# kisasexypantera94/hpfw

Hardware: AMD Instinct MI355X
Metric: hashprints/sec (index) + Hamming matches/sec (search), 30 s@44.1 kHz clips (higher is better)
Workload: dtype f32 (transforms, dB) + int8 digits / int64 sums (projection); 1 GPU; configs[1]: 1000 x 30 s synthetic 44.1 kHz PCM16 clips per GPU, hashprint extraction only (CQT + dB + projection + bit pack), inputs resident in HBM; clips_per_gpu=1000, hashprints_per_clip=2320, parallelism=clips sharded over 1 GPU(s), no collective on this path

## Files before the change

hpfw_amd/csrc/extract.hip:

```cpp
#include "handle.h"

int pass_clips(hpfw_gpu *h, const DevPlan *dp, int64_t n_clips)
{
    const hpfw::HostPlan &p = dp->hp;
    size_t per_clip = (size_t)121 * p.c * 4 + (size_t)64 * std::max(p.n_frames, 1) * 4;
    if (p.bluestein)
        per_clip += 2 * hpfw::bz_plane_bytes(dp->bz, 1) + (size_t)(p.kmax - p.kmin) * 8;
    else
        per_clip += (size_t)hpfw::z_floats_per_clip(p.hq, p.n2) * 4 + (size_t)p.n1 * p.q2w * 8;
    size_t work = 0;
    for (const hpfw::CqClassDev &cd : dp->cls) work = std::max(work, hpfw::cq_big_work_bytes(cd, 1));
    per_clip += work;
    const int64_t fit = std::max<int64_t>(1, (int64_t)(((size_t)24 << 30) / per_clip));
    const int64_t cap = std::min<int64_t>(h->batch, fit), n = std::max<int64_t>(n_clips, 1);
    const int64_t passes = (n + cap - 1) / cap;
    return (int)((n + passes - 1) / passes);
}

int ensure_ws(hpfw_gpu *h, const DevPlan *dp, int nb, int ns)
{
    const hpfw::HostPlan &p = dp->hp;
    size_t work = 0;
    for (const hpfw::CqClassDev &cd : dp->cls) work = std::max(work, hpfw::cq_big_work_bytes(cd, nb));
    if (work) {
// ... 196 lines not shown
{
    *use = nullptr;
    if (n_shifts || h->q_products != 6 || !h->projection) return 0;
    const int64_t tiles = hpfw::project_q_tiles(n_clips, c);
    if (tiles <= 0) return 0;
    if (int rc = ensure(h->d_q_split, hpfw::project_q_split_bytes(tiles, h->q_fixup_launch), h)) return rc;
    *qs = {h->d_q_thr.as<int32_t>(), h->d_q_split.get(), h->q_fixup_launch ? h->d_fq32.as<int32_t>() : nullptr};
    *use = qs;
    return 0;
}

namespace {
int run_back(hpfw_gpu *h, DevPlan *dp, const void *images, int n_shifts, int ns, uint64_t *d_hp, hipStream_t s)
{
    const hpfw::HostPlan &p = dp->hp;
    const float *sdb = h->ws[2].as<float>();
    int rc;
    if (h->projection) {
        hpfw::QSplit qs;
        const hpfw::QSplit *split;
        if ((rc = q_split(h, n_shifts, ns, p.c, &qs, &split))) return rc;
        {
            Timed t(h, K_PROJECT, s);
            hpfw::launch_hashprints_q(images, n_shifts, sdb, h->d_clipmax.as<float>(), ns, p.c, d_hp, nullptr, s, split);
        }
        if (split) h->q_last_tiles = hpfw::project_q_tiles(ns, p.c);
        return check_launch("project");
    }
    float *proj = h->ws[3].as<float>();
    {
        Timed t(h, K_PROJECT, s);
        hpfw::launch_project(h->d_fpack.as<float>(), sdb, h->d_clipmax.as<float>(), ns, p.c, proj, s);
    }
    if ((rc = check_launch("project"))) return rc;
    {
        Timed t(h, K_PACK, s);
        hpfw::launch_pack(proj, ns, p.n_frames, d_hp, s);
    }
    return check_launch("delta_pack");
}

constexpr int kBackBatch = 1024;

int check_filters(const hpfw_gpu *h) { return h->has_filters ? 0 : fail(HPFW_E_NOFILTERS, "no filters: call hpfw_gpu_set_filters or hpfw_gpu_learn_filters first"); }

int check_shifts(const int32_t *shifts, int n_shifts)
{
// ... 30 lines not shown
    if ((rc = check_filters(h))) return rc;
    return 0;
}

int hashprints_from_db(hpfw_gpu *h, const float *d_db, int64_t n_clips, int64_t c, const int32_t *shifts, int n_shifts, uint64_t *d_hp,
                       hipStream_t s)
{
    const int64_t nf = c - (hpfw::kCtx - 1), nhp = nf - hpfw::kLag;
    HIP_TRY(hipSetDevice(h->device));
    return ordered_call(h, s, [&] {
        int rc;
        if (n_shifts && (rc = shift_images(h, shifts, n_shifts, s))) return rc;
        const void *images = n_shifts ? h->d_shift_images.get() : h->d_fq_image.get();
        const int nbmax = 256;
        if (!h->projection && (rc = ensure(h->ws[3], (size_t)nbmax * 64 * (size_t)nf * 4))) return rc;
        hpfw::QSplit qs;
        const hpfw::QSplit *split;
        if ((rc = q_split(h, n_shifts, std::min<int64_t>(nbmax, n_clips), c, &qs, &split))) return rc;
        for (int64_t c0 = 0; c0 < n_clips; c0 += nbmax) {
            const int nb = (int)std::min<int64_t>(nbmax, n_clips - c0);
            if (h->projection) {
                Timed t(h, K_PROJECT, s);
                hpfw::launch_hashprints_q(images, n_shifts, d_db + c0 * 121 * c, nullptr, nb, (int)c, d_hp + c0 * std::max(n_shifts, 1) * nhp,
                                          nullptr, s, split);
                if (split) h->q_last_tiles = hpfw::project_q_tiles(nb, c);
            } else {
                hpfw::launch_project(h->d_fpack.as<float>(), d_db + c0 * 121 * c, nullptr, nb, (int)c, h->ws[3].as<float>(), s);
                hpfw::launch_pack(h->ws[3].as<float>(), nb, (int)nf, d_hp + c0 * nhp, s);
            }
            if ((rc = check_launch("project"))) return rc;
        }
        return 0;
    });
}

constexpr size_t kTempoBudget = (size_t)256 << 20;

int check_tempos(const float *tempos, int n_tempos, int n_shifts)
{
    if (!tempos || n_tempos < 1 || n_tempos > hpfw::kMaxTempos) return fail(HPFW_E_INVALID, "tempos: 1 to 64 values");
    for (int i = 0; i < n_tempos; ++i) {
        if (!(tempos[i] >= 0.5f && tempos[i] <= 2.0f)) return fail(HPFW_E_INVALID, "tempos: finite values in [0.5, 2]");
        for (int j = 0; j < i; ++j)
            if (hpfw::tempo_step(tempos[j]) == hpfw::tempo_step(tempos[i]))
                return fail(HPFW_E_INVALID, "tempos: values must have distinct steps rint(65536 / tempo)");
    }
    if ((int64_t)n_tempos * std::max(n_shifts, 1) > hpfw::kMaxShifts) return fail(HPFW_E_INVALID, "tempos x shifts: at most 64 variants");
// ... 20 lines not shown
    return ct;
}

int tempo_back(hpfw_gpu *h, const void *images, int n_shifts, const float *d_db, int64_t nb, int64_t c, const hpfw::TempoList &tl,
               int64_t ct, uint64_t *d_hp, hipStream_t s)
{
    const int64_t per_pair = (int64_t)std::max(n_shifts, 1) * (ct - (hpfw::kCtx - 1) - hpfw::kLag);
    const size_t pair_bytes = (size_t)hpfw::kBins * ct * 4;
    const int64_t pairs = std::max<int64_t>(1, (int64_t)(kTempoBudget / pair_bytes));
    const int64_t cb = pairs >= tl.n ? std::min<int64_t>(pairs / tl.n, nb) : 1;
    const int tb = pairs >= tl.n ? tl.n : (int)pairs;
    int rc;
    if ((rc = ensure(h->d_tempo, (size_t)cb * tb * pair_bytes, h))) return rc;
    float *scaled = h->d_tempo.as<float>();
    for (int64_t c0 = 0; c0 < nb; c0 += cb) {
        const int nc = (int)std::min(cb, nb - c0);
        for (int j0 = 0; j0 < tl.n; j0 += tb) {
            hpfw::TempoList sub{std::min(tb, tl.n - j0), {}};
            for (int j = 0; j < sub.n; ++j) sub.step[j] = tl.step[j0 + j];
            hpfw::launch_tempo_scale(d_db + c0 * hpfw::kBins * c, nc, c, sub, ct, scaled, s);
            if ((rc = check_launch("tempo_scale"))) return rc;
            {
                Timed t(h, K_PROJECT, s);
                hpfw::launch_hashprints_q(images, n_shifts, scaled, nullptr, nc * sub.n, (int)ct, d_hp + (c0 * tl.n + j0) * per_pair, nullptr, s);
            }
            if ((rc = check_launch("project"))) return rc;
        }
    }
    return 0;
}

int extract_tempo_pcm16(hpfw_gpu *h, const int16_t *d_pcm, int64_t n_samples, int64_t n_clips, const float *tempos, int n_tempos,
                        const int32_t *shifts, int n_shifts, uint64_t *d_hp, void *stream)
{
    hpfw::TempoList tl;
    int rc = check_tempo_call(h, tempos, n_tempos, shifts, n_shifts, &tl);
    if (rc) return rc;
    if (!d_pcm || !d_hp || n_clips < 0) return fail(HPFW_E_INVALID, "bad argument");
    HIP_TRY(hipSetDevice(h->device));
    DevPlan *dp;
    if ((rc = get_plan(h, n_samples, &dp))) return rc;
    const int64_t c = dp->hp.c, ct = tempo_common_columns(c, tl);
    if (ct - (hpfw::kCtx - 1) - hpfw::kLag < 1) return fail(HPFW_E_UNSUPPORTED, "clip too short to yield a hashprint at the slowest tempo");
    if (n_clips == 0) return 0;
    const int64_t per_clip = (int64_t)tl.n * std::max(n_shifts, 1) * (ct - (hpfw::kCtx - 1) - hpfw::kLag);
    hipStream_t s = (hipStream_t)stream;
    return ordered_call(h, s, [&] {
// ... 105 lines not shown
    *tiles = h->q_last_tiles;
    for (uint32_t v : counts) {
        if (v == 0xffffffffu) *redone += 1;
        else *listed += v;
    }
    return 0;
}

int hpfw_gpu_stage_delta_q(hpfw_gpu *h, const float *d_db, int64_t n_clips, int64_t c, int64_t *d_delta, uint64_t *d_hp, void *stream)
{
    if (!h || !d_db || !d_delta) return fail(HPFW_E_INVALID, "null argument");
    if (int rc = check_filters(h)) return rc;
    const int64_t nhp = c - (hpfw::kCtx - 1) - hpfw::kLag;
    if (nhp <= 0 || n_clips <= 0) return 0;
    if (n_clips > 65535) return fail(HPFW_E_INVALID, "at most 65535 clips per call");
    HIP_TRY(hipSetDevice(h->device));
    hipStream_t s = (hipStream_t)stream;
    return ordered_call(h, s, [&] {
        uint64_t *hp = d_hp;
        if (!hp) {
            if (int rc = ensure(h->ws[3], (size_t)n_clips * (size_t)nhp * 8)) return rc;
            hp = h->ws[3].as<uint64_t>();
        }
        hpfw::launch_hashprints_q(h->d_fq_image.get(), 0, d_db, nullptr, (int)n_clips, (int)c, hp, (long long *)d_delta, s);
        return check_launch("project");
    });
}

int hpfw_gpu_hashprints_from_db_transposed(hpfw_gpu *h, const float *d_db, int64_t n_clips, int64_t c, const int32_t *shifts,
                                           int n_shifts, uint64_t *d_hp, void *stream)
{
    int rc = check_transposed(h, shifts, n_shifts);
    if (rc) return rc;
    if (!d_db || !d_hp || n_clips < 0) return fail(HPFW_E_INVALID, "bad argument");
    if (c - (hpfw::kCtx - 1) - hpfw::kLag <= 0 || n_clips == 0) return 0;
    return hashprints_from_db(h, d_db, n_clips, c, shifts, n_shifts, d_hp, (hipStream_t)stream);
}

int hpfw_gpu_extract_pcm16(hpfw_gpu *h, const int16_t *d_pcm, int64_t n_samples, int64_t n_clips,
                           uint64_t *d_hp, void *stream)
{
    return extract_pcm16(h, d_pcm, n_samples, n_clips, nullptr, 0, d_hp, stream);
}

int hpfw_gpu_extract_transposed_pcm16(hpfw_gpu *h, const int16_t *d_pcm, int64_t n_samples, int64_t n_clips, const int32_t *shifts,
                                      int n_shifts, uint64_t *d_hp, void *stream)
{
// ... 440 lines not shown
```

hpfw_amd/csrc/handle.h:

```cpp
#pragma once
#include <hip/hip_runtime.h>

#include <algorithm>
#include <cstdio>
#include <cstdlib>
#include <cstring>
#include <condition_variable>
#include <chrono>
#include <map>
#include <memory>
#include <mutex>
#include <set>
#include <string>
#include <vector>

#include "../../include/hpfw_gpu.h"
#include "combiner.h"
#include "hip_owned.h"
#include "kernels.h"
#include "legacy_internal.h"
#include "plan.h"

using hpfw::DevBuf, hpfw::Event, hpfw::HostBuf, hpfw::Stream;

// ... 29 lines not shown
struct PlanTiming;

enum KernelKind { K_ROWS = 0, K_COLS, K_CQ, K_DB, K_PROJECT, K_PACK, K_SCAN, K_TOPK, K_PAIRS, K_FWD, K_COUNT };

struct TimedLaunch {
    int kind;
    Event a, b;
};

struct CallStatus {
    int rc = 0;
    std::string msg;
};

struct hpfw_gpu {
    int device = 0;
    bool has_filters = false;
    std::vector<float> filters;
    DevBuf d_fpack;
    DevBuf d_fq_image;
    DevBuf d_q_thr, d_fq32, d_q_split;
    int q_products = 6;
    bool q_fixup_launch = false;
    int64_t q_last_tiles = 0;
    int projection = 1;
    struct PlanCache {
        PlanCache();
        ~PlanCache();
        std::multimap<size_t, DevBuf> dev_pool;
        size_t dev_pool_bytes = 0;
        std::map<int64_t, std::unique_ptr<DevPlan>> plans;
        std::mutex host_mtx;
        std::condition_variable host_cv;
        std::map<int64_t, std::unique_ptr<hpfw::HostPlan>> host_ready;
        std::set<int64_t> host_seen;
        size_t plan_bytes = 0;
        uint64_t plan_clock = 0;
        uint64_t idle_clock = 0;
        std::unique_ptr<PlanTiming> plan_timing;
        Stream plan_stream;
        HostBuf pin_ring;
        size_t pin_off = 0;
        Event plan_ev;
        bool plan_ev_pending = false;
    } cache;
    unsigned conventions = 0;
// ... 179 lines not shown
```

hpfw_amd/csrc/handle.hip:

```cpp
#include "handle.h"

namespace {
thread_local std::string g_err;

const char *const kKernelNames[K_COUNT] = {"fwd_rows", "fwd_cols", "cq_chirpz", "db",
                                           "project_mfma", "delta_pack", "hamming_scan", "topk", "pcm_pairs", "fwd_span"};
}

int fail(int code, const std::string &msg)
{
    g_err = msg;
    return code;
}

extern "C" {

const char *hpfw_gpu_last_error(void) { return g_err.c_str(); }
void hpfw_internal_set_error(const char *msg) { g_err = msg ? msg : ""; }
const char *hpfw_gpu_version(void) { return "hpfw-gpu 0.1 (gfx950)"; }

int hpfw_gpu_create(int device, hpfw_gpu **out)
{
    if (!out) return fail(HPFW_E_INVALID, "out is NULL");
    *out = nullptr;
    int n = 0;
    HIP_TRY(hipGetDeviceCount(&n));
    if (device < 0 || device >= n) return fail(HPFW_E_INVALID, "no such device");
    HIP_TRY(hipSetDevice(device));
    auto h = std::make_unique<hpfw_gpu>();
    h->device = device;
    if (std::getenv("HPFW_CQ_SERIAL")) h->cq_concurrent = 0;
    if (const char *e = std::getenv("HPFW_FWD_CHUNK")) h->fwd_chunk = std::max(0, atoi(e));
    if (const char *e = std::getenv("HPFW_BZ_CHUNK")) h->bz_chunk = std::max(0, atoi(e));
    if (const char *e = std::getenv("HPFW_COLS_VARIANT")) h->cols_variant = atoi(e);
    if (const char *e = std::getenv("HPFW_PRUNE")) h->prune = (unsigned)std::strtoul(e, nullptr, 0);
    if (const char *e = std::getenv("HPFW_Q_PRODUCTS")) h->q_products = atoi(e) == 9 ? 9 : 6;
    if (const char *e = std::getenv("HPFW_Q_FIXUP")) h->q_fixup_launch = std::strcmp(e, "launch") == 0;
    if (const char *e = std::getenv("HPFW_DB_TERM")) h->db_fast = std::strcmp(e, "spec") != 0;
    if (const char *e = std::getenv("HPFW_FWD_STREAMS")) h->fwd_streams = std::min(hpfw_gpu::kCqSide + 1, std::max(1, atoi(e)));
    if (const char *e = std::getenv("HPFW_PROJECTION"))
        h->projection = std::strcmp(e, "f32") == 0 ? 0 : 1;
    if (h->ev0.create(hipEventDefault) != hipSuccess || h->ev1.create(hipEventDefault) != hipSuccess || h->order_ev.create() != hipSuccess ||
        init_plans(h.get()) != hipSuccess)
        return fail(HPFW_E_HIP, "hipEventCreate failed");
    *out = h.release();
    return 0;
}

int hpfw_gpu_device(const hpfw_gpu *h) { return h ? h->device : -1; }

void hpfw_gpu_destroy(hpfw_gpu *h)
{
    if (!h) return;
    (void)hipSetDevice(h->device);
    (void)hipDeviceSynchronize();
    delete h;
}

int hpfw_gpu_set_filters(hpfw_gpu *h, const float *f)
{
// ... 111 lines not shown
```

hpfw_amd/csrc/k_project_q.hip:

```cpp
#include <algorithm>
#include <cmath>
#include <cstdint>
#include <cstdlib>
#include <vector>

#include "kernels.h"

namespace hpfw {

extern __shared__ __align__(16) unsigned char smem_raw[];

typedef int v4i __attribute__((ext_vector_type(4)));
typedef int v16i __attribute__((ext_vector_type(16)));

constexpr int kQThreads = 256;
constexpr int kQTileN = 128;
constexpr int kQCols = kQTileN + kCtx - 1;
constexpr int kQPitch = 160;
constexpr int kQChunks = 8;
constexpr int kQUnit = 48;
constexpr int kQSlabBytes = kQChunks * kQPitch * kQUnit;
constexpr int kQStepBytes = 3 * 64 * 16;
constexpr int kQSteps = 2 * kCtx;
constexpr int kQLdsBytes = kQSlabBytes + kQTileN * 4 * 2;
constexpr float kQScale = 98304.0f;
constexpr int kQCap = 128;
constexpr unsigned kQRedo = 0xffffffffu;
constexpr int kQLdsBytes6 = kQLdsBytes + 16;
constexpr int kQLdsBytes6f = kQLdsBytes6 + kQCap * 2;

__device__ __forceinline__ unsigned q_digit_bytes(int u) { return ((unsigned)u + 0x808080u) ^ 0x808080u; }

__device__ __forceinline__ int q_fixed(float s)
{
    return (int)__builtin_rintf(__builtin_fminf(__builtin_fmaxf(s, -80.0f), 0.0f) * kQScale);
}

__device__ __forceinline__ long long q_value_from_digits(const v4i *__restrict__ fq_image, const unsigned char *slab, int r, int nl, int lane)
{
    constexpr int kPairs = 4 * kQSteps;
    v4i fa[3][3], sb[3][3];
#pragma unroll
    for (int k = 0; k < 3; ++k) {
        const int pair = min(lane + 64 * k, kPairs - 1);
        const int s = pair >> 2, g = pair & 3;
        const v4i *fu = fq_image + ((size_t)(r >> 4) * kQSteps + s) * (kQStepBytes / 16) + (r & 15) + 16 * g;
        const v4i *su = reinterpret_cast<const v4i *>(slab + (size_t)((4 * (s & 1) + g) * kQPitch + nl + (s >> 1)) * kQUnit);
#pragma unroll
        for (int d = 0; d < 3; ++d) {
            fa[k][d] = fu[d * 64];
            sb[k][d] = su[d];
        }
    }
    if (lane + 128 >= kPairs) sb[2][0] = sb[2][1] = sb[2][2] = v4i{0, 0, 0, 0};
    int acc[5] = {0, 0, 0, 0, 0};
#pragma unroll
    for (int k = 0; k < 3; ++k)
#pragma unroll
        for (int i = 0; i < 3; ++i)
#pragma unroll
            for (int j = 0; j < 3; ++j)
#pragma unroll
                for (int w = 0; w < 4; ++w) acc[i + j] = __builtin_amdgcn_sdot4(fa[k][i][w], sb[k][j][w], acc[i + j], false);
    long long v = acc[4];
#pragma unroll
    for (int cls = 3; cls >= 0; --cls) v = v * 256 + acc[cls];
#pragma unroll
    for (int m = 32; m >= 1; m >>= 1) v += __shfl_xor(v, m);
    return v;
}

template <bool FROM_T, bool SHIFTED, int NP, bool FUSED = false, bool STAGED = false>
__device__ __forceinline__ void hashprint_q_tile(const unsigned t, const v4i *__restrict__ fq_images, const float *__restrict__ sdb,
                                                 const float *__restrict__ tmax, int c, int nhp, int n_tiles_x, uint64_t *__restrict__ hp,
                                                 long long *__restrict__ dbg, int n_images, const int *__restrict__ thr,
                                                 unsigned *__restrict__ counts, unsigned short *__restrict__ seg)
{
    static_assert(NP == 9 || (NP == 6 && !SHIFTED), "six products: the extraction's unshifted image only");
    static_assert((!FUSED || NP == 6) && (!STAGED || (NP == 9 && !SHIFTED)), "FUSED: six products; STAGED: its nine-product redo");
    unsigned char *slab = smem_raw;
    unsigned short *parts = reinterpret_cast<unsigned short *>(smem_raw + kQSlabBytes);
    unsigned *n_open = reinterpret_cast<unsigned *>(smem_raw + kQLdsBytes);
    unsigned short *list = reinterpret_cast<unsigned short *>(smem_raw + kQLdsBytes6);
    const int tid = threadIdx.x, lane = tid & 63, wave = tid >> 6;
    const int kg = lane >> 4, cl = lane & 15;
    const int clip = t / n_tiles_x;
    const int n0 = (t - clip * n_tiles_x) * kQTileN;
    if (NP == 6 && tid == 0) *n_open = 0;
#if defined(HPFW_Q_STAMPS)
    long long st[6];
    st[0] = __builtin_amdgcn_s_memtime();
#define Q_STAMP(k) st[k] = __builtin_amdgcn_s_memtime()
#else
#define Q_STAMP(k) ((void)0)
#endif
    const float *S = sdb + (int64_t)clip * kBins * c;
    const float ref = FROM_T ? tmax[clip] : 0.0f;
    const v4i *img = fq_images + (size_t)wave * kQSteps * (kQStepBytes / 16) + lane;
    v4i a[3][3];
#pragma unroll
    for (int d = 0; d < 3; ++d) {
        a[0][d] = img[d * 64];
        a[1][d] = img[(kQStepBytes / 16) + d * 64];
    }
    constexpr int kUnits = (kQChunks * kQCols + kQThreads - 1) / kQThreads;
    unsigned any_digit = 0;
#pragma unroll 1
    for (int r0 = STAGED ? kUnits : 0; r0 < kUnits; r0 += 2) {
        float va[2][16], vb[2][16];
#pragma unroll
        for (int rr = 0; rr < 2; ++rr) {
            const int unit = tid + (r0 + rr) * kQThreads;
            const int q = unit / kQCols, col = unit - q * kQCols;
            const int gc = n0 + col;
            const bool in = r0 + rr < kUnits && unit < kQChunks * kQCols && gc + kLag < c;
#pragma unroll
            for (int e = 0; e < 16; ++e) {
                const int bin = 16 * q + e;
                const bool ok = in && bin < kBins;
                const unsigned idx = ok ? (unsigned)(bin * c + gc) : 0u;
                va[rr][e] = S[idx];
                vb[rr][e] = S[idx + kLag];
            }
        }
#pragma unroll
        for (int rr = 0; rr < 2; ++rr) {
            const int unit = tid + (r0 + rr) * kQThreads;
            const int q = unit / kQCols, col = unit - q * kQCols;
            const bool in = r0 + rr < kUnits && unit < kQChunks * kQCols && n0 + col + kLag < c;
#pragma unroll
            for (int e = 0; e < 16; ++e) {
// ... 121 lines not shown
                long long v = acc[f][4][reg];
#pragma unroll
                for (int cls = 3; cls >= (NP == 9 ? 0 : 2); --cls) v = v * 256 + acc[f][cls][reg];
                bits |= (unsigned)(v >= 0) << (15 - row);
                if (NP == 6 && f < n_tiles && n < nhp && (v < 0 ? -v : v) <= (long long)th[reg]) {
                    const unsigned pos = atomicAdd(n_open, 1u);
                    if (pos < (unsigned)kQCap)
                        (FUSED ? list : seg + (size_t)t * kQCap)[pos] = (unsigned short)(((16 * wave + row) << 7) | (16 * f + cl));
                }
#if !defined(HPFW_Q_STAMPS)
                if (!SHIFTED && dbg && f < n_tiles && n < nhp) dbg[((int64_t)clip * kFilters + 16 * wave + row) * nhp + n] = v;
#endif
            }
            bits |= (unsigned)__shfl_xor((int)bits, 16);
            bits |= (unsigned)__shfl_xor((int)bits, 32);
            if (kg == 0) parts[(16 * f + cl) * 4 + wave] = (unsigned short)bits;
        }
        Q_STAMP(4);
        __syncthreads();
        if (FUSED) {
            const unsigned cnt = *n_open;
            if (cnt > (unsigned)kQCap) {
                if (tid == 0) counts[t] = kQRedo;
                hashprint_q_tile<FROM_T, false, 9, false, true>(t, fq_images, sdb, tmax, c, nhp, n_tiles_x, hp, nullptr, 1, nullptr, nullptr, nullptr);
                return;
            }
            if (cnt > 0) {
                for (unsigned e = (unsigned)__builtin_amdgcn_readfirstlane(wave); e < cnt; e += kQThreads / 64) {
                    const int entry = __builtin_amdgcn_readfirstlane((int)list[e]);
                    const int r = entry >> 7, nl = entry & 127;
                    const long long d = q_value_from_digits(fq_images, slab, r, nl, lane);
                    if (lane == 0) {
                        unsigned *w = reinterpret_cast<unsigned *>(parts) + nl * 2 + (r >> 5);
                        const unsigned bit = 1u << (16 * ((r >> 4) & 1) + 15 - (r & 15));
                        if (((*static_cast<volatile unsigned *>(w) & bit) != 0) != (d >= 0)) atomicXor(w, bit);
                    }
                }
                __syncthreads();
            }
        }
        if (tid < kQTileN && n0 + tid < nhp) {
            const unsigned short *p = parts + tid * 4;
            hp[((int64_t)clip * (SHIFTED ? n_images : 1) + im) * nhp + n0 + tid] =
                ((uint64_t)p[0] << 48) | ((uint64_t)p[1] << 32) | ((uint64_t)p[2] << 16) | (uint64_t)p[3];
        }
        if (NP == 6 && tid == 0) counts[t] = *n_open <= (unsigned)kQCap ? *n_open : kQRedo;
    } while (SHIFTED && ++im < n_images);
#if defined(HPFW_Q_STAMPS)
    Q_STAMP(5);
    if (dbg && tid == 0) {
        for (int k = 0; k < 6; ++k) dbg[(int64_t)t * 8 + k] = st[k];
        dbg[(int64_t)t * 8 + 6] = __builtin_amdgcn_s_getreg((15 << 11) | 4);
        dbg[(int64_t)t * 8 + 7] = blockIdx.x;
    }
#endif
}

__device__ __forceinline__ unsigned q_tile_of_workgroup()
{
    const unsigned per_xcd = (gridDim.x + 7) / 8;
    return (blockIdx.x & 7) * per_xcd + (blockIdx.x >> 3);
}

template <bool FROM_T, bool SHIFTED>
__global__ __launch_bounds__(kQThreads, 2) void hashprint_q_kernel(const v4i *__restrict__ fq_images, const float *__restrict__ sdb,
                                                                   const float *__restrict__ tmax, int c, int nhp, int n_tiles_x, int n_clips,
                                                                   uint64_t *__restrict__ hp, long long *__restrict__ dbg, int n_images)
{
    const unsigned t = q_tile_of_workgroup();
    if (t >= (unsigned)(n_tiles_x * n_clips)) return;
    hashprint_q_tile<FROM_T, SHIFTED, 9>(t, fq_images, sdb, tmax, c, nhp, n_tiles_x, hp, dbg, n_images, nullptr, nullptr, nullptr);
}

template <bool FROM_T>
__global__ __launch_bounds__(kQThreads, 2) void hashprint_q6_kernel(const v4i *__restrict__ fq_image, const float *__restrict__ sdb,
                                                                    const float *__restrict__ tmax, int c, int nhp, int n_tiles_x, int n_clips,
                                                                    uint64_t *__restrict__ hp, const int *__restrict__ thr,
                                                                    unsigned *__restrict__ counts)
{
    const unsigned t = q_tile_of_workgroup();
    if (t >= (unsigned)(n_tiles_x * n_clips)) return;
    hashprint_q_tile<FROM_T, false, 6, true>(t, fq_image, sdb, tmax, c, nhp, n_tiles_x, hp, nullptr, 1, thr, counts, nullptr);
}

template <bool FROM_T>
__global__ __launch_bounds__(kQThreads, 2) void hashprint_q6_listed_kernel(const v4i *__restrict__ fq_image, const float *__restrict__ sdb,
                                                                           const float *__restrict__ tmax, int c, int nhp, int n_tiles_x,
                                                                           int n_clips, uint64_t *__restrict__ hp, const int *__restrict__ thr,
                                                                           unsigned *__restrict__ counts, unsigned short *__restrict__ seg)
{
    const unsigned t = q_tile_of_workgroup();
    if (t >= (unsigned)(n_tiles_x * n_clips)) return;
    hashprint_q_tile<FROM_T, false, 6>(t, fq_image, sdb, tmax, c, nhp, n_tiles_x, hp, nullptr, 1, thr, counts, seg);
}

template <bool FROM_T>
__global__ __launch_bounds__(kQThreads, 2) void hashprint_q_fixup_kernel(const v4i *__restrict__ fq_image, const int *__restrict__ fq32,
                                                                         const float *__restrict__ sdb, const float *__restrict__ tmax, int c,
                                                                         int nhp, int n_tiles_x, int n_clips, uint64_t *__restrict__ hp,
                                                                         const unsigned *__restrict__ counts,
                                                                         const unsigned short *__restrict__ seg)
{
    const int lane = threadIdx.x & 63, wave = threadIdx.x >> 6;
    const unsigned total = (unsigned)(n_tiles_x * n_clips);
    for (unsigned t = blockIdx.x; t < total; t += gridDim.x) {
        const unsigned cnt = counts[t];
        if (cnt == 0) continue;
        if (cnt == kQRedo) {
            __syncthreads();
            hashprint_q_tile<FROM_T, false, 9>(t, fq_image, sdb, tmax, c, nhp, n_tiles_x, hp, nullptr, 1, nullptr, nullptr, nullptr);
            continue;
        }
        const int clip = t / n_tiles_x;
        const int n0 = (t - clip * n_tiles_x) * kQTileN;
        const float *S = sdb + (int64_t)clip * kBins * c;
        const float ref = FROM_T ? tmax[clip] : 0.0f;
        for (unsigned e = wave; e < cnt; e += kQThreads / 64) {
            const unsigned entry = seg[(size_t)t * kQCap + e];
            const int r = entry >> 7, n = n0 + (int)(entry & 127u);
            const int *frow = fq32 + r * kFrame;
            long long sum = 0;
#pragma unroll 2
            for (int k = lane; k < kFrame; k += 64) {
                const int bin = k / kCtx, idx = bin * c + n + (k - bin * kCtx);
                float xa = S[idx], xb = S[idx + kLag];
                if (FROM_T) {
                    xa -= ref;
                    xb -= ref;
                }
                sum += (long long)frow[k] * (long long)(q_fixed(xa) - q_fixed(xb));
            }
#pragma unroll
            for (int m = 32; m >= 1; m >>= 1) sum += __shfl_xor(sum, m);
// ... 50 lines not shown
            }
            const int64_t lmax = 128 * (s0 + 256 * (s0 + s1));
            thr->push_back(lmax > 0 ? (int32_t)(lmax >> 16) : -1);
        }
    }
    image.assign((size_t)4 * kQSteps * kQStepBytes, 0);
    for (int w = 0; w < 4; ++w)
        for (int t = 0; t < kCtx; ++t)
            for (int p = 0; p < 2; ++p)
                for (int l = 0; l < 64; ++l)
                    for (int e = 0; e < 16; ++e) {
                        const int bin = 64 * p + 16 * (l >> 4) + e;
                        if (bin >= kBins) continue;
                        const int u = fq[(size_t)(16 * w + (l & 15)) * kFrame + bin * kCtx + t];
                        const int d0 = ((u + 128) & 255) - 128, u1 = (u - d0) >> 8, d1 = ((u1 + 128) & 255) - 128, d2 = (u1 - d1) >> 8;
                        const int d[3] = {d0, d1, d2};
                        for (int i = 0; i < 3; ++i)
                            image[((size_t)w * kQSteps + (2 * t + p)) * kQStepBytes + ((size_t)i * 64 + l) * 16 + e] = (int8_t)d[i];
                    }
}

#if defined(HPFW_Q_STAMPS)
static long long *g_q_stamps = nullptr;
extern "C" void hpfw_gpu_debug_set_q_stamps(void *d) { g_q_stamps = static_cast<long long *>(d); }
#endif

size_t project_q_image_bytes() { return (size_t)4 * kQSteps * kQStepBytes; }
size_t project_q_split_bytes(int64_t tiles, bool segments) { return (size_t)tiles * (4 + (segments ? (size_t)kQCap * 2 : 0)); }
int64_t project_q_tiles(int64_t n_clips, int64_t c)
{
    const int64_t nhp = c - (kCtx - 1) - kLag;
    return nhp > 0 ? n_clips * ((nhp + kQTileN - 1) / kQTileN) : 0;
}

void launch_hashprints_q(const void *d_images, int n_shifts, const float *d_db, const float *d_tmax, int n_clips, int c, uint64_t *d_hp,
                         long long *d_dbg, hipStream_t s, const QSplit *split)
{
    static PerDeviceOnce attr_set;
    if (attr_set.need()) {
        for (const void *k : {reinterpret_cast<const void *>(hashprint_q_kernel<true, false>), reinterpret_cast<const void *>(hashprint_q_kernel<false, false>),
                              reinterpret_cast<const void *>(hashprint_q_kernel<true, true>), reinterpret_cast<const void *>(hashprint_q_kernel<false, true>)})
            (void)hipFuncSetAttribute(k, hipFuncAttributeMaxDynamicSharedMemorySize, kQLdsBytes);
        for (const void *k : {reinterpret_cast<const void *>(hashprint_q6_listed_kernel<true>), reinterpret_cast<const void *>(hashprint_q6_listed_kernel<false>),
                              reinterpret_cast<const void *>(hashprint_q_fixup_kernel<true>), reinterpret_cast<const void *>(hashprint_q_fixup_kernel<false>)})
            (void)hipFuncSetAttribute(k, hipFuncAttributeMaxDynamicSharedMemorySize, kQLdsBytes6);
        for (const void *k : {reinterpret_cast<const void *>(hashprint_q6_kernel<true>), reinterpret_cast<const void *>(hashprint_q6_kernel<false>)})
            (void)hipFuncSetAttribute(k, hipFuncAttributeMaxDynamicSharedMemorySize, kQLdsBytes6f);
        attr_set.mark();
    }
    const int nhp = c - (kCtx - 1) - kLag;
    if (nhp <= 0 || n_clips <= 0 || n_shifts < 0) return;
#if defined(HPFW_Q_STAMPS)
    if (!d_dbg) d_dbg = g_q_stamps;
#endif
    const int tiles = (nhp + kQTileN - 1) / kQTileN;
    const dim3 grid(8 * (unsigned)(((int64_t)tiles * n_clips + 7) / 8));
    if (split && n_shifts == 0 && !d_dbg) {
        const int *fq32 = split->d_fq32, *thr = split->d_thr;
        unsigned *counts = static_cast<unsigned *>(split->d_work);
        if (!fq32) {
            hipLaunchKernelGGL(d_tmax ? hashprint_q6_kernel<true> : hashprint_q6_kernel<false>, grid, dim3(kQThreads), kQLdsBytes6f, s,
                               static_cast<const v4i *>(d_images), d_db, d_tmax, c, nhp, tiles, n_clips, d_hp, thr, counts);
            return;
        }
        unsigned short *seg = reinterpret_cast<unsigned short *>(counts + (size_t)tiles * n_clips);
        hipLaunchKernelGGL(d_tmax ? hashprint_q6_listed_kernel<true> : hashprint_q6_listed_kernel<false>, grid, dim3(kQThreads), kQLdsBytes6, s,
                           static_cast<const v4i *>(d_images), d_db, d_tmax, c, nhp, tiles, n_clips, d_hp, thr, counts, seg);
        const unsigned fix = (unsigned)std::min<int64_t>((int64_t)tiles * n_clips, 2048);
        hipLaunchKernelGGL(d_tmax ? hashprint_q_fixup_kernel<true> : hashprint_q_fixup_kernel<false>, dim3(fix), dim3(kQThreads), kQLdsBytes6, s,
                           static_cast<const v4i *>(d_images), fq32, d_db, d_tmax, c, nhp, tiles, n_clips, d_hp, counts, seg);
        return;
    }
    auto k = n_shifts > 0 ? (d_tmax ? hashprint_q_kernel<true, true> : hashprint_q_kernel<false, true>)
                          : (d_tmax ? hashprint_q_kernel<true, false> : hashprint_q_kernel<false, false>);
    hipLaunchKernelGGL(k, grid, dim3(kQThreads), kQLdsBytes, s, static_cast<const v4i *>(d_images), d_db, d_tmax, c, nhp, tiles, n_clips,
                       d_hp, d_dbg, n_shifts);
}

void launch_shift_filter_images(const void *d_fq_image, const ShiftList &shifts, void *d_images, hipStream_t s)
{
    constexpr int kUnits = 4 * kQSteps * kQStepBytes / 16;
    hipLaunchKernelGGL(shift_filter_images_kernel, dim3((kUnits + 255) / 256, shifts.n), dim3(256), 0, s,
                       static_cast<const unsigned char *>(d_fq_image), shifts, static_cast<v4i *>(d_images));
}

}
```

hpfw_amd/csrc/kernels.h:

```cpp
#pragma once
#include <cmath>
#include <cstdint>
#include <vector>
#include <atomic>
#include <hip/hip_runtime.h>
#include <stdint.h>

#include "../../include/hpfw_gpu.h"
#include "device_math.h"
#include "fft_lds.h"
#include "fft_rows.h"
#include "streams_plan.h"
#include "xcorr_plan.h"

namespace hpfw {

struct PerDeviceOnce {
    std::atomic<uint64_t> done{0};
    static uint64_t bit()
    {
        int dev = 0;
        (void)hipGetDevice(&dev);
        return 1ull << (dev & 63);
    }
// ... 163 lines not shown
                     float *d_mag, float *d_wavemax, int db_mode, hipStream_t s);
size_t cq_big_work_bytes(const CqClassDev &cc, int n_clips);
void launch_cq_big_class(const CqPlanDev &cp, const CqClassDev &cc, const cf *d_x, int n_clips, cf *d_work, float *d_mag,
                         float *d_wavemax, int db_mode, hipStream_t s);
void launch_clipmax(const float *d_wavemax, float *d_clipmax, int n_clips, hipStream_t s);
void launch_db_finish(float *d_t, const float *d_clipmax, int n_clips, int64_t per_clip, hipStream_t s);
void launch_magmax(const float *d_mag, int n_clips, int c, float *d_wavemax, hipStream_t s);
void launch_db(const float *d_mag, const float *d_wavemax, float *d_clipmax, int n_clips, int64_t per_clip,
               float *d_db, bool fast, hipStream_t s);
void launch_db_term_sweep(uint32_t first, uint64_t count, unsigned long long *d_out, hipStream_t s);
void launch_project(const float *d_fpack, const float *d_db, const float *d_tmax, int n_clips, int c,
                    float *d_proj, hipStream_t s);
void launch_pack(const float *d_proj, int n_clips, int nf, uint64_t *d_hp, hipStream_t s);
size_t project_q_image_bytes();
struct QSplit {
    const int32_t *d_thr;
    void *d_work;
    const int32_t *d_fq32;
};
size_t project_q_split_bytes(int64_t tiles, bool segments);
int64_t project_q_tiles(int64_t n_clips, int64_t c);
void pack_filters_q(const float *f_colmajor, std::vector<int8_t> &image, std::vector<int32_t> *thr = nullptr, std::vector<int32_t> *fq32 = nullptr);
void launch_hashprints_q(const void *d_images, int n_shifts, const float *d_db, const float *d_tmax, int n_clips, int c, uint64_t *d_hp,
                         long long *d_dbg, hipStream_t s, const QSplit *split = nullptr);
constexpr int kMaxShifts = 64;
struct ShiftList {
    int n;
    int s[kMaxShifts];
};
void launch_shift_filter_images(const void *d_fq_image, const ShiftList &shifts, void *d_images, hipStream_t s);
constexpr int kMaxTempos = 64;
struct TempoList {
    int n;
    int32_t step[kMaxTempos];
};
inline int32_t tempo_step(float rho) { return (int32_t)std::rint(65536.0 / (double)rho); }
inline int64_t tempo_columns(int64_t c, int32_t step) { return (c - 1) * 65536 / step + 1; }
void launch_tempo_scale(const float *d_db, int n_clips, int64_t c, const TempoList &tl, int64_t ct, float *d_out, hipStream_t s);

struct CfgArgs {
    int rows, context, lag, filters;
    const float *fpack;
};
size_t cfg_fpack_floats(int rows, int context, int filters);
void pack_cfg_filters(int rows, int context, int filters, const float *f_colmajor, float *fpack);
size_t project_cfg_lds_bytes(const CfgArgs &a);
void launch_project_cfg(const CfgArgs &a, const float *d_s, const int *d_cols, int n_clips, int64_t stride, float *d_proj,
// ... 104 lines not shown
```

Before: 299.0 million hashprints/s.

## Software-pipeline projection staging loads and remap short last tiles in grid

Replaces the default staging loop of the quantised projection kernel with a task-based scheme: each thread issues dB loads two tasks ahead, then quantises the three columns into digit differences and writes byte-plane vectors to LDS using perm instructions. It also changes the workgroup-to-tile mapping so short final tiles of each clip are scheduled as a separate XCD-interleaved group, with the grid sized to match. The goal is to hide global load latency during staging and balance uneven tiles across XCDs. The old path is kept behind HPFW_Q_STAGING=classic. The added register arrays may raise register pressure and reduce occupancy.

```diff
diff --git a/hpfw_amd/csrc/extract.hip b/hpfw_amd/csrc/extract.hip
--- a/hpfw_amd/csrc/extract.hip
+++ b/hpfw_amd/csrc/extract.hip
@@ -242,7 +242,7 @@
         if ((rc = q_split(h, n_shifts, ns, p.c, &qs, &split))) return rc;
         {
             Timed t(h, K_PROJECT, s);
-            hpfw::launch_hashprints_q(images, n_shifts, sdb, h->d_clipmax.as<float>(), ns, p.c, d_hp, nullptr, s, split);
+            hpfw::launch_hashprints_q(images, n_shifts, sdb, h->d_clipmax.as<float>(), ns, p.c, d_hp, nullptr, s, split, h->q_staging_classic);
         }
         if (split) h->q_last_tiles = hpfw::project_q_tiles(ns, p.c);
         return check_launch("project");
@@ -319,7 +319,7 @@
             if (h->projection) {
                 Timed t(h, K_PROJECT, s);
                 hpfw::launch_hashprints_q(images, n_shifts, d_db + c0 * 121 * c, nullptr, nb, (int)c, d_hp + c0 * std::max(n_shifts, 1) * nhp,
-                                          nullptr, s, split);
+                                          nullptr, s, split, h->q_staging_classic);
                 if (split) h->q_last_tiles = hpfw::project_q_tiles(nb, c);
             } else {
                 hpfw::launch_project(h->d_fpack.as<float>(), d_db + c0 * 121 * c, nullptr, nb, (int)c, h->ws[3].as<float>(), s);
@@ -386,7 +386,8 @@
             if ((rc = check_launch("tempo_scale"))) return rc;
             {
                 Timed t(h, K_PROJECT, s);
-                hpfw::launch_hashprints_q(images, n_shifts, scaled, nullptr, nc * sub.n, (int)ct, d_hp + (c0 * tl.n + j0) * per_pair, nullptr, s);
+                hpfw::launch_hashprints_q(images, n_shifts, scaled, nullptr, nc * sub.n, (int)ct, d_hp + (c0 * tl.n + j0) * per_pair, nullptr, s, nullptr,
+                                          h->q_staging_classic);
             }
             if ((rc = check_launch("project"))) return rc;
         }
@@ -538,7 +539,7 @@
             if (int rc = ensure(h->ws[3], (size_t)n_clips * (size_t)nhp * 8)) return rc;
             hp = h->ws[3].as<uint64_t>();
         }
-        hpfw::launch_hashprints_q(h->d_fq_image.get(), 0, d_db, nullptr, (int)n_clips, (int)c, hp, (long long *)d_delta, s);
+        hpfw::launch_hashprints_q(h->d_fq_image.get(), 0, d_db, nullptr, (int)n_clips, (int)c, hp, (long long *)d_delta, s, nullptr, h->q_staging_classic);
         return check_launch("project");
     });
 }
diff --git a/hpfw_amd/csrc/handle.h b/hpfw_amd/csrc/handle.h
--- a/hpfw_amd/csrc/handle.h
+++ b/hpfw_amd/csrc/handle.h
@@ -75,6 +75,7 @@
     DevBuf d_q_thr, d_fq32, d_q_split;
     int q_products = 6;
     bool q_fixup_launch = false;
+    bool q_staging_classic = false;
     int64_t q_last_tiles = 0;
     int projection = 1;
     struct PlanCache {
diff --git a/hpfw_amd/csrc/handle.hip b/hpfw_amd/csrc/handle.hip
--- a/hpfw_amd/csrc/handle.hip
+++ b/hpfw_amd/csrc/handle.hip
@@ -36,6 +36,7 @@
     if (const char *e = std::getenv("HPFW_PRUNE")) h->prune = (unsigned)std::strtoul(e, nullptr, 0);
     if (const char *e = std::getenv("HPFW_Q_PRODUCTS")) h->q_products = atoi(e) == 9 ? 9 : 6;
     if (const char *e = std::getenv("HPFW_Q_FIXUP")) h->q_fixup_launch = std::strcmp(e, "launch") == 0;
+    if (const char *e = std::getenv("HPFW_Q_STAGING")) h->q_staging_classic = std::strcmp(e, "classic") == 0;
     if (const char *e = std::getenv("HPFW_DB_TERM")) h->db_fast = std::strcmp(e, "spec") != 0;
     if (const char *e = std::getenv("HPFW_FWD_STREAMS")) h->fwd_streams = std::min(hpfw_gpu::kCqSide + 1, std::max(1, atoi(e)));
     if (const char *e = std::getenv("HPFW_PROJECTION"))
diff --git a/hpfw_amd/csrc/k_project_q.hip b/hpfw_amd/csrc/k_project_q.hip
--- a/hpfw_amd/csrc/k_project_q.hip
+++ b/hpfw_amd/csrc/k_project_q.hip
@@ -10,6 +10,7 @@
 
 extern __shared__ __align__(16) unsigned char smem_raw[];
 
+typedef int v2i __attribute__((ext_vector_type(2)));
 typedef int v4i __attribute__((ext_vector_type(4)));
 typedef int v16i __attribute__((ext_vector_type(16)));
 
@@ -31,9 +32,29 @@
 
 __device__ __forceinline__ unsigned q_digit_bytes(int u) { return ((unsigned)u + 0x808080u) ^ 0x808080u; }
 
+#if defined(HPFW_Q_STAMPS)
+__device__ long long *g_q_stamps_dev = nullptr;
+#endif
+
 __device__ __forceinline__ int q_fixed(float s)
 {
     return (int)__builtin_rintf(__builtin_fminf(__builtin_fmaxf(s, -80.0f), 0.0f) * kQScale);
+}
+
+constexpr int kQHeavy = kQCols - kLag;
+constexpr int kQTasks = 2 * kQChunks * kLag / kQThreads;
+constexpr int kQAhead = 2;
+static_assert(kQTasks * kQThreads == 2 * kQChunks * kLag && kQHeavy > 0 && kQHeavy <= kLag, "1280 tasks, five per thread");
+
+__device__ __forceinline__ void q_planes(const unsigned (&w)[4], unsigned (&p)[3])
+{
+    const unsigned t01 = __builtin_amdgcn_perm(w[1], w[0], 0x05010400u);
+    const unsigned t23 = __builtin_amdgcn_perm(w[3], w[2], 0x05010400u);
+    const unsigned u01 = __builtin_amdgcn_perm(w[1], w[0], 0x0c0c0602u);
+    const unsigned u23 = __builtin_amdgcn_perm(w[3], w[2], 0x0c0c0602u);
+    p[0] = __builtin_amdgcn_perm(t23, t01, 0x05040100u);
+    p[1] = __builtin_amdgcn_perm(t23, t01, 0x07060302u);
+    p[2] = __builtin_amdgcn_perm(u23, u01, 0x05040100u);
 }
 
 __device__ __forceinline__ long long q_value_from_digits(const v4i *__restrict__ fq_image, const unsigned char *slab, int r, int nl, int lane)
@@ -70,7 +91,7 @@
     return v;
 }
 
-template <bool FROM_T, bool SHIFTED, int NP, bool FUSED = false, bool STAGED = false>
+template <bool FROM_T, bool SHIFTED, int NP, bool CLASSIC, bool FUSED = false, bool STAGED = false>
 __device__ __forceinline__ void hashprint_q_tile(const unsigned t, const v4i *__restrict__ fq_images, const float *__restrict__ sdb,
                                                  const float *__restrict__ tmax, int c, int nhp, int n_tiles_x, uint64_t *__restrict__ hp,
                                                  long long *__restrict__ dbg, int n_images, const int *__restrict__ thr,
@@ -103,10 +124,66 @@
         a[0][d] = img[d * 64];
         a[1][d] = img[(kQStepBytes / 16) + d * 64];
     }
+    unsigned any_digit = 0;
+    if constexpr (!CLASSIC && !STAGED) {
+        float x[kQTasks][3][8];
+        auto issue = [&](int i) {
+            const int task = tid + i * kQThreads, qh = task / kLag, r = task - qh * kLag;
+            const int gc = n0 + r;
+            const bool in0 = gc + kLag < c, in1 = r < kQHeavy && gc + 2 * kLag < c;
+#pragma unroll
+            for (int e = 0; e < 8; ++e) {
+                const int bin = 8 * qh + e;
+                const unsigned at = (unsigned)(bin * c + gc);
+                const unsigned i0 = in0 && bin < kBins ? at : 0u, i2 = in1 && bin < kBins ? at + 2 * kLag : 0u;
+                x[i][0][e] = S[i0];
+                x[i][1][e] = S[i0 + kLag];
+                x[i][2][e] = S[i2];
+            }
+        };
+        auto quantise = [&](int i) {
+            const int task = tid + i * kQThreads, qh = task / kLag, r = task - qh * kLag;
+            const int gc = n0 + r;
+            const bool in0 = gc + kLag < c, in1 = r < kQHeavy && gc + 2 * kLag < c;
+            unsigned wa[8], wb[8];
+#pragma unroll
+            for (int e = 0; e < 8; ++e) {
+                const bool okb = 8 * qh + e < kBins;
+                float x0 = x[i][0][e], x1 = x[i][1][e], x2 = x[i][2][e];
+                if (FROM_T) {
+                    x0 -= ref;
+                    x1 -= ref;
+                    x2 -= ref;
+                }
+                const int u0 = q_fixed(x0), u1 = q_fixed(x1), u2 = q_fixed(x2);
+                wa[e] = q_digit_bytes(in0 && okb ? u0 - u1 : 0);
+                wb[e] = q_digit_bytes(in1 && okb ? u1 - u2 : 0);
+            }
+            unsigned char *dst = slab + (size_t)((qh >> 1) * kQPitch + r) * kQUnit + 8 * (qh & 1);
+            auto store = [&](const unsigned (&w)[8], unsigned char *to) {
+                unsigned lo[3], hi[3];
+                q_planes({w[0], w[1], w[2], w[3]}, lo);
+                q_planes({w[4], w[5], w[6], w[7]}, hi);
+#pragma unroll
+                for (int j = 0; j < 3; ++j) *reinterpret_cast<v2i *>(to + 16 * j) = v2i{(int)lo[j], (int)hi[j]};
+                if (NP == 6) any_digit |= lo[0] | lo[1] | lo[2] | hi[0] | hi[1] | hi[2];
+            };
+            static_assert(kLag + kLag <= kQPitch, "spare columns for the chains' unconditional second store");
+            store(wa, dst);
+            store(wb, dst + (size_t)kLag * kQUnit);
+        };
+#pragma unroll
+        for (int i = 0; i < kQAhead && i < kQTasks; ++i) issue(i);
+#pragma unroll
+        for (int i = 0; i < kQTasks; ++i) {
+            if (i + kQAhead < kQTasks) issue(i + kQAhead);
+            __builtin_amdgcn_sched_barrier(0);
+            quantise(i);
+        }
+    }
     constexpr int kUnits = (kQChunks * kQCols + kQThreads - 1) / kQThreads;
-    unsigned any_digit = 0;
 #pragma unroll 1
-    for (int r0 = STAGED ? kUnits : 0; r0 < kUnits; r0 += 2) {
+    for (int r0 = STAGED || !CLASSIC ? kUnits : 0; r0 < kUnits; r0 += 2) {
         float va[2][16], vb[2][16];
 #pragma unroll
         for (int rr = 0; rr < 2; ++rr) {
@@ -274,7 +351,8 @@
             const unsigned cnt = *n_open;
             if (cnt > (unsigned)kQCap) {
                 if (tid == 0) counts[t] = kQRedo;
-                hashprint_q_tile<FROM_T, false, 9, false, true>(t, fq_images, sdb, tmax, c, nhp, n_tiles_x, hp, nullptr, 1, nullptr, nullptr, nullptr);
+                hashprint_q_tile<FROM_T, false, 9, CLASSIC, false, true>(t, fq_images, sdb, tmax, c, nhp, n_tiles_x, hp, nullptr, 1, nullptr, nullptr,
+                                                                         nullptr);
                 return;
             }
             if (cnt > 0) {
@@ -300,50 +378,75 @@
     } while (SHIFTED && ++im < n_images);
 #if defined(HPFW_Q_STAMPS)
     Q_STAMP(5);
-    if (dbg && tid == 0) {
-        for (int k = 0; k < 6; ++k) dbg[(int64_t)t * 8 + k] = st[k];
-        dbg[(int64_t)t * 8 + 6] = __builtin_amdgcn_s_getreg((15 << 11) | 4);
-        dbg[(int64_t)t * 8 + 7] = blockIdx.x;
+    long long *stamps = dbg ? dbg : g_q_stamps_dev;
+    if (stamps && tid == 0 && !STAGED) {
+        for (int k = 0; k < 6; ++k) stamps[(int64_t)t * 8 + k] = st[k];
+        stamps[(int64_t)t * 8 + 6] = __builtin_amdgcn_s_getreg((15 << 11) | 4);
+        stamps[(int64_t)t * 8 + 7] = blockIdx.x;
     }
 #endif
 }
 
-__device__ __forceinline__ unsigned q_tile_of_workgroup()
-{
-    const unsigned per_xcd = (gridDim.x + 7) / 8;
-    return (blockIdx.x & 7) * per_xcd + (blockIdx.x >> 3);
-}
-
-template <bool FROM_T, bool SHIFTED>
+constexpr unsigned kQNoTile = 0xffffffffu;
+__host__ __device__ inline bool q_short_last(int nhp, int n_tiles_x) { return nhp - (n_tiles_x - 1) * kQTileN <= kQTileN - 16; }
+__host__ __device__ inline unsigned q_round8(unsigned n) { return 8 * ((n + 7) / 8); }
+
+static unsigned q_grid(bool classic, int nhp, int n_tiles_x, int n_clips)
+{
+    if (classic || !q_short_last(nhp, n_tiles_x)) return q_round8((unsigned)n_tiles_x * (unsigned)n_clips);
+    return q_round8((unsigned)(n_tiles_x - 1) * (unsigned)n_clips) + q_round8((unsigned)n_clips);
+}
+
+template <bool CLASSIC>
+__device__ __forceinline__ unsigned q_tile_of_workgroup(int nhp, int n_tiles_x, int n_clips)
+{
+    unsigned b = blockIdx.x;
+    if (CLASSIC || !q_short_last(nhp, n_tiles_x)) {
+        const unsigned t = (b & 7) * (gridDim.x / 8) + (b >> 3);
+        return t < (unsigned)(n_tiles_x * n_clips) ? t : kQNoTile;
+    }
+    const unsigned full_x = (unsigned)(n_tiles_x - 1), n_full = full_x * (unsigned)n_clips, grid_full = q_round8(n_full);
+    if (b < grid_full) {
+        const unsigned j = (b & 7) * (grid_full / 8) + (b >> 3);
+        if (j >= n_full) return kQNoTile;
+        const unsigned clip = j / full_x;
+        return clip * (unsigned)n_tiles_x + (j - clip * full_x);
+    }
+    b -= grid_full;
+    const unsigned j = (b & 7) * ((gridDim.x - grid_full) / 8) + (b >> 3);
+    return j < (unsigned)n_clips ? j * (unsigned)n_tiles_x + full_x : kQNoTile;
+}
+
+template <bool FROM_T, bool SHIFTED, bool CLASSIC>
 __global__ __launch_bounds__(kQThreads, 2) void hashprint_q_kernel(const v4i *__restrict__ fq_images, const float *__restrict__ sdb,
                                                                    const float *__restrict__ tmax, int c, int nhp, int n_tiles_x, int n_clips,
                                                                    uint64_t *__restrict__ hp, long long *__restrict__ dbg, int n_images)
 {
-    const unsigned t = q_tile_of_workgroup();
-    if (t >= (unsigned)(n_tiles_x * n_clips)) return;
-    hashprint_q_tile<FROM_T, SHIFTED, 9>(t, fq_images, sdb, tmax, c, nhp, n_tiles_x, hp, dbg, n_images, nullptr, nullptr, nullptr);
-}
-
-template <bool FROM_T>
+    const unsigned t = q_tile_of_workgroup<CLASSIC>(nhp, n_tiles_x, n_clips);
+    if (t == kQNoTile) return;
+    hashprint_q_tile<FROM_T, SHIFTED, 9, CLASSIC>(t, fq_images, sdb, tmax, c, nhp, n_tiles_x, hp, dbg, n_images, nullptr, nullptr, nullptr);
+}
+
+template <bool FROM_T, bool CLASSIC>
 __global__ __launch_bounds__(kQThreads, 2) void hashprint_q6_kernel(const v4i *__restrict__ fq_image, const float *__restrict__ sdb,
                                                                     const float *__restrict__ tmax, int c, int nhp, int n_tiles_x, int n_clips,
                                                                     uint64_t *__restrict__ hp, const int *__restrict__ thr,
                                                                     unsigned *__restrict__ counts)
 {
-    const unsigned t = q_tile_of_workgroup();
-    if (t >= (unsigned)(n_tiles_x * n_clips)) return;
-    hashprint_q_tile<FROM_T, false, 6, true>(t, fq_image, sdb, tmax, c, nhp, n_tiles_x, hp, nullptr, 1, thr, counts, nullptr);
-}
-
-template <bool FROM_T>
+    const unsigned t = q_tile_of_workgroup<CLASSIC>(nhp, n_tiles_x, n_clips);
+    if (t == kQNoTile) return;
+    hashprint_q_tile<FROM_T, false, 6, CLASSIC, true>(t, fq_image, sdb, tmax, c, nhp, n_tiles_x, hp, nullptr, 1, thr, counts, nullptr);
+}
+
+template <bool FROM_T, bool CLASSIC>
 __global__ __launch_bounds__(kQThreads, 2) void hashprint_q6_listed_kernel(const v4i *__restrict__ fq_image, const float *__restrict__ sdb,
                                                                            const float *__restrict__ tmax, int c, int nhp, int n_tiles_x,
                                                                            int n_clips, uint64_t *__restrict__ hp, const int *__restrict__ thr,
                                                                            unsigned *__restrict__ counts, unsigned short *__restrict__ seg)
 {
-    const unsigned t = q_tile_of_workgroup();
-    if (t >= (unsigned)(n_tiles_x * n_clips)) return;
-    hashprint_q_tile<FROM_T, false, 6>(t, fq_image, sdb, tmax, c, nhp, n_tiles_x, hp, nullptr, 1, thr, counts, seg);
+    const unsigned t = q_tile_of_workgroup<CLASSIC>(nhp, n_tiles_x, n_clips);
+    if (t == kQNoTile) return;
+    hashprint_q_tile<FROM_T, false, 6, CLASSIC>(t, fq_image, sdb, tmax, c, nhp, n_tiles_x, hp, nullptr, 1, thr, counts, seg);
 }
 
 template <bool FROM_T>
@@ -360,7 +463,7 @@
         if (cnt == 0) continue;
         if (cnt == kQRedo) {
             __syncthreads();
-            hashprint_q_tile<FROM_T, false, 9>(t, fq_image, sdb, tmax, c, nhp, n_tiles_x, hp, nullptr, 1, nullptr, nullptr, nullptr);
+            hashprint_q_tile<FROM_T, false, 9, true>(t, fq_image, sdb, tmax, c, nhp, n_tiles_x, hp, nullptr, 1, nullptr, nullptr, nullptr);
             continue;
         }
         const int clip = t / n_tiles_x;
@@ -457,7 +560,11 @@
 
 #if defined(HPFW_Q_STAMPS)
 static long long *g_q_stamps = nullptr;
-extern "C" void hpfw_gpu_debug_set_q_stamps(void *d) { g_q_stamps = static_cast<long long *>(d); }
+extern "C" void hpfw_gpu_debug_set_q_stamps(void *d)
+{
+    g_q_stamps = static_cast<long long *>(d);
+    (void)hipMemcpyToSymbol(HIP_SYMBOL(g_q_stamps_dev), &g_q_stamps, sizeof(g_q_stamps));
+}
 #endif
 
 size_t project_q_image_bytes() { return (size_t)4 * kQSteps * kQStepBytes; }
@@ -468,48 +575,63 @@
     return nhp > 0 ? n_clips * ((nhp + kQTileN - 1) / kQTileN) : 0;
 }
 
-void launch_hashprints_q(const void *d_images, int n_shifts, const float *d_db, const float *d_tmax, int n_clips, int c, uint64_t *d_hp,
-                         long long *d_dbg, hipStream_t s, const QSplit *split)
+template <bool CLASSIC>
+static void launch_hashprints_q_as(const void *d_images, int n_shifts, const float *d_db, const float *d_tmax, int n_clips, int c, uint64_t *d_hp,
+                                   long long *d_dbg, hipStream_t s, const QSplit *split)
 {
     static PerDeviceOnce attr_set;
     if (attr_set.need()) {
-        for (const void *k : {reinterpret_cast<const void *>(hashprint_q_kernel<true, false>), reinterpret_cast<const void *>(hashprint_q_kernel<false, false>),
-                              reinterpret_cast<const void *>(hashprint_q_kernel<true, true>), reinterpret_cast<const void *>(hashprint_q_kernel<false, true>)})
+        for (const void *k :
+             {reinterpret_cast<const void *>(hashprint_q_kernel<true, false, CLASSIC>), reinterpret_cast<const void *>(hashprint_q_kernel<false, false, CLASSIC>),
+              reinterpret_cast<const void *>(hashprint_q_kernel<true, true, CLASSIC>), reinterpret_cast<const void *>(hashprint_q_kernel<false, true, CLASSIC>)})
             (void)hipFuncSetAttribute(k, hipFuncAttributeMaxDynamicSharedMemorySize, kQLdsBytes);
-        for (const void *k : {reinterpret_cast<const void *>(hashprint_q6_listed_kernel<true>), reinterpret_cast<const void *>(hashprint_q6_listed_kernel<false>),
-                              reinterpret_cast<const void *>(hashprint_q_fixup_kernel<true>), reinterpret_cast<const void *>(hashprint_q_fixup_kernel<false>)})
+        for (const void *k :
+             {reinterpret_cast<const void *>(hashprint_q6_listed_kernel<true, CLASSIC>), reinterpret_cast<const void *>(hashprint_q6_listed_kernel<false, CLASSIC>),
+              reinterpret_cast<const void *>(hashprint_q_fixup_kernel<true>), reinterpret_cast<const void *>(hashprint_q_fixup_kernel<false>)})
             (void)hipFuncSetAttribute(k, hipFuncAttributeMaxDynamicSharedMemorySize, kQLdsBytes6);
-        for (const void *k : {reinterpret_cast<const void *>(hashprint_q6_kernel<true>), reinterpret_cast<const void *>(hashprint_q6_kernel<false>)})
+        for (const void *k : {reinterpret_cast<const void *>(hashprint_q6_kernel<true, CLASSIC>), reinterpret_cast<const void *>(hashprint_q6_kernel<false, CLASSIC>)})
             (void)hipFuncSetAttribute(k, hipFuncAttributeMaxDynamicSharedMemorySize, kQLdsBytes6f);
         attr_set.mark();
     }
     const int nhp = c - (kCtx - 1) - kLag;
     if (nhp <= 0 || n_clips <= 0 || n_shifts < 0) return;
 #if defined(HPFW_Q_STAMPS)
-    if (!d_dbg) d_dbg = g_q_stamps;
+    if (!d_dbg && !(split && n_shifts == 0)) d_dbg = g_q_stamps;
 #endif
     const int tiles = (nhp + kQTileN - 1) / kQTileN;
-    const dim3 grid(8 * (unsigned)(((int64_t)tiles * n_clips + 7) / 8));
+    const dim3 grid(q_grid(CLASSIC, nhp, tiles, n_clips));
     if (split && n_shifts == 0 && !d_dbg) {
         const int *fq32 = split->d_fq32, *thr = split->d_thr;
         unsigned *counts = static_cast<unsigned *>(split->d_work);
         if (!fq32) {
-            hipLaunchKernelGGL(d_tmax ? hashprint_q6_kernel<true> : hashprint_q6_kernel<false>, grid, dim3(kQThreads), kQLdsBytes6f, s,
-                               static_cast<const v4i *>(d_images), d_db, d_tmax, c, nhp, tiles, n_clips, d_hp, thr, counts);
+            auto k6 = d_tmax ? hashprint_q6_kernel<true, CLASSIC> : hashprint_q6_kernel<false, CLASSIC>;
+            hipLaunchKernelGGL(k6, grid, dim3(kQThreads), kQLdsBytes6f, s, static_cast<const v4i *>(d_images), d_db, d_tmax, c, nhp, tiles, n_clips,
+                               d_hp, thr, counts);
             return;
         }
         unsigned short *seg = reinterpret_cast<unsigned short *>(counts + (size_t)tiles * n_clips);
-        hipLaunchKernelGGL(d_tmax ? hashprint_q6_listed_kernel<true> : hashprint_q6_listed_kernel<false>, grid, dim3(kQThreads), kQLdsBytes6, s,
-                           static_cast<const v4i *>(d_images), d_db, d_tmax, c, nhp, tiles, n_clips, d_hp, thr, counts, seg);
+        auto k6 = d_tmax ? hashprint_q6_listed_kernel<true, CLASSIC> : hashprint_q6_listed_kernel<false, CLASSIC>;
+        hipLaunchKernelGGL(k6, grid, dim3(kQThreads), kQLdsBytes6, s, static_cast<const v4i *>(d_images), d_db, d_tmax, c, nhp, tiles, n_clips,
+                           d_hp, thr, counts, seg);
         const unsigned fix = (unsigned)std::min<int64_t>((int64_t)tiles * n_clips, 2048);
-        hipLaunchKernelGGL(d_tmax ? hashprint_q_fixup_kernel<true> : hashprint_q_fixup_kernel<false>, dim3(fix), dim3(kQThreads), kQLdsBytes6, s,
-                           static_cast<const v4i *>(d_images), fq32, d_db, d_tmax, c, nhp, tiles, n_clips, d_hp, counts, seg);
+        auto kf = d_tmax ? hashprint_q_fixup_kernel<true> : hashprint_q_fixup_kernel<false>;
+        hipLaunchKernelGGL(kf, dim3(fix), dim3(kQThreads), kQLdsBytes6, s, static_cast<const v4i *>(d_images), fq32, d_db, d_tmax, c, nhp, tiles,
+                           n_clips, d_hp, counts, seg);
         return;
     }
-    auto k = n_shifts > 0 ? (d_tmax ? hashprint_q_kernel<true, true> : hashprint_q_kernel<false, true>)
-                          : (d_tmax ? hashprint_q_kernel<true, false> : hashprint_q_kernel<false, false>);
+    auto k = n_shifts > 0 ? (d_tmax ? hashprint_q_kernel<true, true, CLASSIC> : hashprint_q_kernel<false, true, CLASSIC>)
+                          : (d_tmax ? hashprint_q_kernel<true, false, CLASSIC> : hashprint_q_kernel<false, false, CLASSIC>);
     hipLaunchKernelGGL(k, grid, dim3(kQThreads), kQLdsBytes, s, static_cast<const v4i *>(d_images), d_db, d_tmax, c, nhp, tiles, n_clips,
                        d_hp, d_dbg, n_shifts);
+}
+
+void launch_hashprints_q(const void *d_images, int n_shifts, const float *d_db, const float *d_tmax, int n_clips, int c, uint64_t *d_hp,
+                         long long *d_dbg, hipStream_t s, const QSplit *split, bool classic_staging)
+{
+    if (classic_staging)
+        launch_hashprints_q_as<true>(d_images, n_shifts, d_db, d_tmax, n_clips, c, d_hp, d_dbg, s, split);
+    else
+        launch_hashprints_q_as<false>(d_images, n_shifts, d_db, d_tmax, n_clips, c, d_hp, d_dbg, s, split);
 }
 
 void launch_shift_filter_images(const void *d_fq_image, const ShiftList &shifts, void *d_images, hipStream_t s)
diff --git a/hpfw_amd/csrc/kernels.h b/hpfw_amd/csrc/kernels.h
--- a/hpfw_amd/csrc/kernels.h
+++ b/hpfw_amd/csrc/kernels.h
@@ -209,7 +209,7 @@
 int64_t project_q_tiles(int64_t n_clips, int64_t c);
 void pack_filters_q(const float *f_colmajor, std::vector<int8_t> &image, std::vector<int32_t> *thr = nullptr, std::vector<int32_t> *fq32 = nullptr);
 void launch_hashprints_q(const void *d_images, int n_shifts, const float *d_db, const float *d_tmax, int n_clips, int c, uint64_t *d_hp,
-                         long long *d_dbg, hipStream_t s, const QSplit *split = nullptr);
+                         long long *d_dbg, hipStream_t s, const QSplit *split = nullptr, bool classic_staging = false);
 constexpr int kMaxShifts = 64;
 struct ShiftList {
     int n;
```

Measured after the change: 302.0 million hashprints/s (median of 6 runs). +1.0%, better.
